# Samirez/Visual_odometry

Hardware: AMD Instinct MI355X
Metric: frame-pairs/sec (1280x720, 2000 ORB feats) (higher is better)
Workload: dtype u8+f32+f64; 1 GPU; seeded synthetic 1280x720 drone flight (256 distinct rendered views, closed loop), 2000 ORB features/frame, 8 levels = BASELINE config 2; chunk of 257 consecutive frames -> 256 pairs (k, k+1) per GPU per step, each frame detected once; detector=orb, distinct_rendered_frames=256, pair_stride=1, contexts_per_gpu=3, keypoint_order=cv2, poly_solver=fast, matcher=crosscheck, matcher_kernel=mfma_fp4, ransac=5-point, conf 0.99, 1 px, seed 2^64-1, <=1000 iters, parallelism=single GPU, pairs_ok_last_step=256

## Files before the change

### include/vo_hip.h

```cpp
#ifndef VO_HIP_H
#define VO_HIP_H
#include <stddef.h>
#include <stdint.h>

#ifdef __cplusplus
extern "C" {
#endif

#define VO_MAX_LEVELS 16

#define VO_OK                 0
#define VO_WARN_CAPACITY      1
#define VO_ERR_INVALID       -1
#define VO_ERR_HIP           -2
#define VO_ERR_TOO_FEW       -3
#define VO_ERR_NO_MODEL      -4
#define VO_ERR_NOT_CONFIGURED -5
#define VO_ERR_UNSUPPORTED    -7
#define VO_ERR_AMBIGUOUS      -6

typedef struct vo_ctx vo_ctx;

typedef struct {
    int32_t nfeatures;
// ... 71 lines not shown
typedef struct {
    int32_t match_mode;
    double  ratio;
    double  ransac_prob;
    double  ransac_thresh;
    int32_t ransac_max_iters;
    uint64_t ransac_seed;
    double  pose_dist_thresh;
    int32_t want_points;
} vo_pair_opts;

typedef struct {
    int32_t n_kp1, n_kp2, n_match, n_inl, n_good, status, ransac_iters, reserved;
    double  R[9], t[3], E[9];
} vo_pair_result;

int vo_batch_configure(vo_ctx* ctx, int h, int w, const vo_orb_params* params, int max_frames, int max_pairs);
int vo_frames_upload(vo_ctx* ctx, const uint8_t* frames, int F, int row_stride, int64_t frame_stride, int first_slot);
int vo_frames_upload_async(vo_ctx* ctx, const uint8_t* frames, int F, int row_stride, int64_t frame_stride, int first_slot);
int vo_frames_upload_color(vo_ctx* ctx, const uint8_t* frames, int F, int channels, int row_stride,
                           int64_t frame_stride, int first_slot);
int vo_frames_detect(vo_ctx* ctx, int first_slot, int F);
int vo_frames_detect_async(vo_ctx* ctx, int first_slot, int F);
int vo_batch_kp_capacity(vo_ctx* ctx);
int  vo_host_alloc(size_t bytes, void** out);
void vo_host_free(void* p);
int vo_frame_features(vo_ctx* ctx, int slot, float* kp_xy, float* kp_size, float* kp_angle, float* kp_response,
                      int32_t* kp_octave, uint8_t* desc, int cap, int32_t* n_out);
int vo_pairs_run(vo_ctx* ctx, const int32_t* pair_slots, int B, const double* K, const vo_pair_opts* opts,
                 vo_pair_result* results, double* X, int32_t x_cap);
int vo_pairs_run_async(vo_ctx* ctx, const int32_t* pair_slots, int B, const double* K, const vo_pair_opts* opts,
                       vo_pair_result* results, double* X, int32_t x_cap);
int vo_sync(vo_ctx* ctx);
int vo_detect_after(vo_ctx* ctx, vo_ctx* other);
int vo_pair_matches(vo_ctx* ctx, int pair, int32_t* qidx, int32_t* tidx, float* dist, uint8_t* inlier_mask,
                    int cap, int32_t* n_out);

#define VO_COMM_ID_BYTES 128
#define VO_RECORD_DOUBLES 16
int vo_comm_unique_id(uint8_t id[VO_COMM_ID_BYTES]);
int vo_comm_init(vo_ctx* ctx, const uint8_t id[VO_COMM_ID_BYTES], int rank, int world);
int vo_comm_destroy(vo_ctx* ctx);
int vo_comm_share(vo_ctx* ctx, vo_ctx* owner);
int vo_comm_info(vo_ctx* ctx, int32_t* n_ranks, int32_t* rank);
int vo_pairs_gather(vo_ctx* ctx, int B, double* gathered, int wait);
int vo_comm_allgather_f64(vo_ctx* ctx, const double* send, int n, double* recv);
// ... 223 lines not shown
```

### visual_odometry_amd/_lib.py

```python
from __future__ import annotations

import ctypes as C
import os

import numpy as np

_HERE = os.path.dirname(os.path.abspath(__file__))
LIB_PATH = os.environ.get("VO_HIP_LIBRARY") or os.path.join(_HERE, "libvo_hip.so")

VO_OK, VO_WARN_CAPACITY = 0, 1
VO_ERR_INVALID, VO_ERR_HIP, VO_ERR_TOO_FEW, VO_ERR_NO_MODEL, VO_ERR_NOT_CONFIGURED, VO_ERR_AMBIGUOUS = -1, -2, -3, -4, -5, -6
VO_ERR_UNSUPPORTED = -7
VO_STAGE_COUNT = 30
VO_COMM_ID_BYTES, VO_RECORD_DOUBLES = 128, 16
VO_BA_MAX_CAMERAS, VO_BA_MAX_FREE = 64, 16
VO_BA_LARGE_MAX_FREE = 512
VO_PGO_MAX_VERTICES, VO_PGO_MAX_LOOPS = 8192, 32
VO_STATS_HIST = 64


class OrbParams(C.Structure):
    _fields_ = [("nfeatures", C.c_int32), ("scale_factor", C.c_float), ("nlevels", C.c_int32),
                ("edge_threshold", C.c_int32), ("first_level", C.c_int32), ("wta_k", C.c_int32),
                ("score_type", C.c_int32), ("patch_size", C.c_int32), ("fast_threshold", C.c_int32)]
# ... 55 lines not shown
    "vo_orb_detect_and_compute": (C.c_int, [_P, _P, C.c_int, C.c_int, C.c_int, C.c_int, _P, _P, _P, _P, _P, _P, _P, C.c_int, _P]),
    "vo_match_hamming": (C.c_int, [_P, _P, C.c_int, _P, C.c_int, C.c_int, _P, _P, _P, _P]),
    "vo_match_l2": (C.c_int, [_P, _P, C.c_int, _P, C.c_int, C.c_int, C.c_int, _P, _P, _P, _P]),
    "vo_knn2_ratio_hamming": (C.c_int, [_P, _P, C.c_int, _P, C.c_int, C.c_double, _P, _P, _P, _P]),
    "vo_find_essential_ransac": (C.c_int, [_P, _P, _P, C.c_int, _P, C.c_double, C.c_double, C.c_int, C.c_uint64, _P, _P, _P, _P]),
    "vo_recover_pose": (C.c_int, [_P, _P, _P, _P, C.c_int, _P, C.c_double, _P, _P, _P, _P]),
    "vo_triangulate": (C.c_int, [_P, _P, _P, _P, _P, C.c_int, _P]),
    "vo_correspond_epilines": (C.c_int, [_P, _P, C.c_int, C.c_int, C.c_int, _P, _P]),
    "vo_pairs_epipolar": (C.c_int, [_P, C.c_int, _P, _P, _P, _P, _P, _P]),
    "vo_undistort_points": (C.c_int, [_P, _P, C.c_int, C.c_int, _P, _P, C.c_int, _P, _P, _P]),
    "vo_frames_undistort": (C.c_int, [_P, C.c_int, C.c_int, _P, _P, C.c_int]),
    "vo_packed_pyramid_bytes": (C.c_int64, [C.c_int, C.c_int, _P]),
    "vo_stage_pyramid": (C.c_int, [_P, _P, C.c_int, C.c_int, C.c_int, C.c_int, _P, _P]),
    "vo_stage_fast_scores": (C.c_int, [_P, _P, C.c_int, C.c_int, C.c_int, C.c_int, _P, _P]),
    "vo_stage_blur": (C.c_int, [_P, _P, C.c_int, C.c_int, C.c_int, C.c_int, _P, _P]),
    "vo_stage_five_point": (C.c_int, [_P, _P, _P, _P, _P]),
    "vo_batch_configure": (C.c_int, [_P, C.c_int, C.c_int, _P, C.c_int, C.c_int]),
    "vo_frames_upload": (C.c_int, [_P, _P, C.c_int, C.c_int, C.c_int64, C.c_int]),
    "vo_frames_upload_async": (C.c_int, [_P, _P, C.c_int, C.c_int, C.c_int64, C.c_int]),
    "vo_frames_upload_color": (C.c_int, [_P, _P, C.c_int, C.c_int, C.c_int, C.c_int64, C.c_int]),
    "vo_frames_detect": (C.c_int, [_P, C.c_int, C.c_int]),
    "vo_frames_detect_async": (C.c_int, [_P, C.c_int, C.c_int]),
    "vo_batch_kp_capacity": (C.c_int, [_P]),
    "vo_host_alloc": (C.c_int, [C.c_size_t, C.POINTER(_P)]),
    "vo_host_free": (None, [_P]),
    "vo_frame_features": (C.c_int, [_P, C.c_int, _P, _P, _P, _P, _P, _P, C.c_int, _P]),
    "vo_pairs_run": (C.c_int, [_P, _P, C.c_int, _P, _P, _P, _P, C.c_int32]),
    "vo_pairs_run_async": (C.c_int, [_P, _P, C.c_int, _P, _P, _P, _P, C.c_int32]),
    "vo_sync": (C.c_int, [_P]),
    "vo_set_matcher_kernel": (C.c_int, [_P, C.c_int]),
    "vo_set_poly_solver": (C.c_int, [_P, C.c_int]),
    "vo_set_pnp_refine": (C.c_int, [_P, C.c_int]),
    "vo_set_keypoint_order": (C.c_int, [_P, C.c_int]),
    "vo_stage_retain_best": (C.c_int, [_P, _P, C.c_int, C.c_int, _P, _P]),
    "vo_detect_after": (C.c_int, [_P, _P]),
    "vo_knn2_hamming": (C.c_int, [_P, _P, C.c_int, _P, C.c_int, _P, _P]),
    "vo_knn2_l2": (C.c_int, [_P, _P, C.c_int, _P, C.c_int, C.c_int, _P, _P]),
    "vo_knn2_ratio_l2": (C.c_int, [_P, _P, C.c_int, _P, C.c_int, C.c_int, C.c_double, _P, _P, _P, _P]),
    "vo_tracks_pnp_batch": (C.c_int, [_P, C.c_int, _P, C.c_int, C.c_double, C.c_double, C.c_uint64, C.c_double, _P, _P, _P, _P, _P]),
    "vo_slam_chain": (C.c_int, [_P, C.c_int, _P, _P, _P, _P, _P, _P, _P, _P, _P, _P, _P, _P, _P]),
    "vo_slam_map_size": (C.c_int, [_P, C.c_int, _P, _P, _P]),
    "vo_slam_map": (C.c_int, [_P, C.c_int, _P, _P, _P, _P, _P, _P, _P, _P]),
    "vo_slam_stream": (C.c_int, [_P, C.c_int, C.c_int, C.c_int, _P, _P, _P, _P, _P, _P, _P, _P, _P, _P, _P, _P, _P, _P, _P, _P]),
    "vo_slam_stream_restart": (C.c_int, [_P, C.c_int, C.c_int, C.c_int, _P, _P, _P, _P, _P, _P, _P, _P, _P, _P, _P, _P, _P, _P, _P, _P, _P, _P, _P, _P]),
    "vo_slam_chains": (C.c_int, [_P, C.c_int, _P, _P, _P, C.c_int, _P, _P, _P, _P, _P, _P, _P, _P, _P, _P, _P]),
    "vo_slam_chains_restart": (C.c_int, [_P, C.c_int, _P, _P, _P, C.c_int, _P, _P, _P, _P, _P, _P, _P, _P, _P, _P, _P, _P, _P, _P, _P]),
# ... 255 lines not shown
```

### visual_odometry_amd/csrc/orb_kernels.hip

```cpp
#include "vo_internal.h"
#include <type_traits>
#include <float.h>
#include <stdlib.h>

__constant__ __attribute__((aligned(16))) int8_t c_pattern[256 * 4] = {
#include "orb_pattern.inc"
};
__constant__ int c_umax[16] = {15, 15, 15, 15, 14, 14, 14, 13, 13, 12, 11, 10, 9, 8, 6, 3};
__constant__ int c_gauss7[7] = {18, 34, 49, 55, 49, 34, 18};


typedef short vo_s16x2 __attribute__((ext_vector_type(2)));
typedef unsigned short vo_u16x2 __attribute__((ext_vector_type(2)));
__device__ __forceinline__ uint32_t pk_sub16(uint32_t a, uint32_t b)
{
    return __builtin_bit_cast(uint32_t, __builtin_bit_cast(vo_s16x2, a) - __builtin_bit_cast(vo_s16x2, b));
}
__device__ __forceinline__ uint32_t pk_add16(uint32_t a, uint32_t b)
{
    return __builtin_bit_cast(uint32_t, __builtin_bit_cast(vo_s16x2, a) + __builtin_bit_cast(vo_s16x2, b));
}
__device__ __forceinline__ uint32_t pk_min16(uint32_t a, uint32_t b)
{
    return __builtin_bit_cast(uint32_t, __builtin_elementwise_min(__builtin_bit_cast(vo_s16x2, a), __builtin_bit_cast(vo_s16x2, b)));
// ... 79 lines not shown
        const int x = x4 + b;
        if (x < w) {
            const uint8_t* px = s + (size_t)x * channels;
            const int v = channels == 1 ? px[0] : (px[0] * 3735 + px[1] * 19235 + px[2] * 9798 + (1 << 14)) >> 15;
            out |= (uint32_t)v << (8 * b);
        }
    }
    if (x4 + 4 <= w && ((dstride | (int)(dframe & 3)) & 3) == 0) *(uint32_t*)d = out;
    else for (int b = 0; b < 4 && x4 + b < w; b++) d[b] = (uint8_t)(out >> (8 * b));
}

void launch_gray_plain(hipStream_t s, const uint8_t* src, int channels, int row_stride, int64_t frame_stride,
                       uint8_t* dst, int w, int h, int dstride, int64_t dframe, int F)
{
    dim3 grid(((w + 3) / 4 + 63) / 64, h, F);
    hipLaunchKernelGGL(k_gray_plain, grid, dim3(64), 0, s, src, channels, row_stride, frame_stride, dst, w, dstride, dframe);
}

__global__ void k_resize(uint8_t* pyr, int frame_bytes, LevelGeom src, LevelGeom dst, ResizeTab tab)
{
    const int f = blockIdx.z;
    const int dx0 = (blockIdx.x * blockDim.x + threadIdx.x) * 4;
    const int dy = blockIdx.y * blockDim.y + threadIdx.y;
    if (dx0 >= dst.stride || dy >= dst.h) return;
    const uint8_t* sp = pyr + (size_t)f * frame_bytes + src.off;
    uint8_t* dp = pyr + (size_t)f * frame_bytes + dst.off;
    int r0, r1; uint32_t w0 = 0, w1 = 0; bool edge;
    if (dy < tab.min_y)       { r0 = r1 = 0; edge = true; }
    else if (dy >= tab.max_y) { r0 = r1 = src.h - 1; edge = true; }
    else { r0 = tab.yofs[dy]; r1 = r0 + 1; edge = false; w1 = tab.yc1[dy]; w0 = 256 - w1; }
    const uint8_t* s0 = sp + (size_t)r0 * src.stride;
    const uint8_t* s1 = sp + (size_t)r1 * src.stride;
    uint32_t out = 0;
#pragma unroll
    for (int b = 0; b < 4; b++) {
        const int dx = dx0 + b;
        uint32_t v = 0;
        if (dx < dst.w) {
            uint32_t h0, h1;
            if (dx < tab.min_x)       { h0 = (uint32_t)s0[0] << 8; h1 = (uint32_t)s1[0] << 8; }
            else if (dx >= tab.max_x) { h0 = (uint32_t)s0[src.w - 1] << 8; h1 = (uint32_t)s1[src.w - 1] << 8; }
            else {
                const int xo = tab.xofs[dx];
                const uint32_t c1 = tab.xc1[dx], c0 = 256 - c1;
                h0 = c0 * s0[xo] + c1 * s0[xo + 1];
                h1 = c0 * s1[xo] + c1 * s1[xo + 1];
            }
            v = edge ? (h0 + 128u) >> 8 : (h0 * w0 + h1 * w1 + 32768u) >> 16;
            v = v > 255u ? 255u : v;
        }
        out |= v << (8 * b);
    }
    *(uint32_t*)(dp + (size_t)dy * dst.stride + dx0) = out;
}

template <int I, int N, typename F>
__device__ __forceinline__ void unroll_while(int n, F& f)
{
    if constexpr (I < N) {
        if (I < n) { f(std::integral_constant<int, I>{}); unroll_while<I + 1, N>(n, f); }
    }
}

#ifndef RS3_AHEAD
#define RS3_AHEAD 4
#endif
__global__ __launch_bounds__(RS2_THREADS) void k_resize_direct(uint8_t* pyr, int frame_bytes, LevelGeom src, LevelGeom dst, ResizeTab tab)
{
    const int f = blockIdx.z, tid = threadIdx.x, lane = tid & 63, wave = __builtin_amdgcn_readfirstlane(tid >> 6);
    const int tiles_x = (dst.w + RS2_WW - 1) / RS2_WW;
    const int bid = xcd_tile(blockIdx.x, gridDim.x);
    const int tx = bid % tiles_x, ty = bid / tiles_x;
    const int x0 = tx * RS2_WW, y0 = ty * RS2_TH;
    const int dy0 = y0 + wave * RS2_WH, dy1 = min(dy0 + RS2_WH, dst.h);
    if (dy0 >= dst.h) return;
    const uint8_t* sp = pyr + (size_t)f * frame_bytes + src.off;
    const int dx = x0 + 4 * lane;
    int o[4], c1[4];
#pragma unroll
    for (int i = 0; i < 4; i++) { const int xi = min(dx + i, dst.w - 1); o[i] = tab.xofs[xi]; c1[i] = tab.xc1[xi]; }
    static_assert(RS2_WH <= 64, "one lane per destination row of the strip");
    const int li = min(dy0 + lane, dst.h - 1);
    const int yo_l = tab.yofs[li];
    const uint32_t yw1 = tab.yc1[li];
    const int yc_l = (int)((256u - yw1) | (yw1 << 16));
    const int yo_first = __builtin_amdgcn_readlane(yo_l, 0), yo_last = __builtin_amdgcn_readlane(yo_l, dy1 - 1 - dy0);
    const int base = o[0] & ~3, sh = o[0] - base;
    const uint32_t q1 = (uint32_t)(o[1] - o[0]), q2 = (uint32_t)(o[2] - o[0]), q3 = (uint32_t)(o[3] - o[0]);
    const uint32_t sel_ae = 0x0c000c00u | (q2 << 16), sel_ao = 0x0c000c00u | q1 | (q3 << 16);
    const uint32_t sel_be = sel_ae + 0x00010001u, sel_bo = sel_ao + 0x00010001u;
    const uint32_t c1e = (uint32_t)c1[0] | ((uint32_t)c1[2] << 16), c1o = (uint32_t)c1[1] | ((uint32_t)c1[3] << 16);
    const int r_first = yo_first, r_end = yo_last + 2;
    static_assert((RS2_WH * 127 + 99) / 100 + 3 <= 32, "the emit mask of a strip fits 32 bits");
    uint32_t emask = dy0 + lane < dy1 ? 1u << (yo_l + 1 - r_first) : 0u;
#pragma unroll
    for (int d = 1; d < RS2_WH; d <<= 1) emask |= (uint32_t)__shfl_xor((int)emask, d, 64);
    emask = (uint32_t)__builtin_amdgcn_readfirstlane((int)emask);
    const __amdgpu_buffer_rsrc_t drs = __builtin_amdgcn_make_buffer_rsrc(pyr + (size_t)f * frame_bytes + dst.off, 0, dst.stride * dst.h, 0x00020000);
    uint32_t out = (uint32_t)(dy0 * dst.stride + dx);
    const bool col_ok = dx < dst.stride;
    const int hmax = src.h - 1;
    uint32_t w[RS3_AHEAD][3];
#pragma unroll
    for (int u = 0; u < RS3_AHEAD; u++) {
        const uint32_t* q = (const uint32_t*)(sp + ((uint32_t)(min(r_first + u, hmax) * src.stride) + (uint32_t)base));
        w[u][0] = q[0]; w[u][1] = q[1]; w[u][2] = q[2];
    }
    int dyi = 0;
    uint32_t pe = 0, po = 0;
    const int nrows = r_end - r_first;
    constexpr int RS3_MAXR = (RS2_WH * 127 + 99) / 100 + 3;
    auto row = [&](auto ic) {
        constexpr int i = decltype(ic)::value, u = i % RS3_AHEAD;
        const uint32_t w0 = w[u][0], w1 = w[u][1], w2 = w[u][2];
        {
            const uint32_t* q = (const uint32_t*)(sp + ((uint32_t)(min(r_first + i + RS3_AHEAD, hmax) * src.stride) + (uint32_t)base));
            w[u][0] = q[0]; w[u][1] = q[1]; w[u][2] = q[2];
        }
        const uint32_t x0w = __builtin_amdgcn_alignbyte(w1, w0, (uint32_t)sh), x1w = __builtin_amdgcn_alignbyte(w2, w1, (uint32_t)sh);
        const uint32_t a_e = __builtin_amdgcn_perm(x1w, x0w, sel_ae), a_o = __builtin_amdgcn_perm(x1w, x0w, sel_ao);
        const uint32_t b_e = __builtin_amdgcn_perm(x1w, x0w, sel_be), b_o = __builtin_amdgcn_perm(x1w, x0w, sel_bo);
        const vo_u16x2 h_e = __builtin_bit_cast(vo_u16x2, c1e) * __builtin_bit_cast(vo_u16x2, pk_sub16(b_e, a_e)) + __builtin_bit_cast(vo_u16x2, a_e << 8);
        const vo_u16x2 h_o = __builtin_bit_cast(vo_u16x2, c1o) * __builtin_bit_cast(vo_u16x2, pk_sub16(b_o, a_o)) + __builtin_bit_cast(vo_u16x2, a_o << 8);
// ... 6 lines not shown
            const uint32_t d2 = __builtin_amdgcn_udot2(__builtin_bit_cast(vo_u16x2, __builtin_amdgcn_perm(ce, pe, 0x07060302u)), wv, 32768u, false);
            const uint32_t d1 = __builtin_amdgcn_udot2(__builtin_bit_cast(vo_u16x2, __builtin_amdgcn_perm(co, po, 0x05040100u)), wv, 32768u, false);
            const uint32_t d3 = __builtin_amdgcn_udot2(__builtin_bit_cast(vo_u16x2, __builtin_amdgcn_perm(co, po, 0x07060302u)), wv, 32768u, false);
            const uint32_t t01 = __builtin_amdgcn_perm(d1, d0, 0x0c0c0602u), t23 = __builtin_amdgcn_perm(d3, d2, 0x0c0c0602u);
            __builtin_amdgcn_raw_buffer_store_b32(__builtin_amdgcn_perm(t23, t01, 0x05040100u), drs, col_ok && emit ? out : 0xfffffff0u, 0, 0);
            out += emit ? (uint32_t)dst.stride : 0u;
            dyi += emit ? 1 : 0;
        }
        pe = ce; po = co;
    };
    unroll_while<0, RS3_MAXR>(nrows, row);
}

void launch_resize(hipStream_t s, uint8_t* pyr, const PyrGeom& g, int level, const ResizeTab& tab, int F)
{
    const LevelGeom& d = g.lv[level];
    if (tab.direct) {
        dim3 grid(((d.w + RS2_WW - 1) / RS2_WW) * ((d.h + RS2_TH - 1) / RS2_TH), 1, F);
        hipLaunchKernelGGL(k_resize_direct, grid, dim3(RS2_THREADS), 0, s, pyr, g.frame_bytes, g.lv[level - 1], d, tab);
        return;
    }
    dim3 block(64, 4), grid((d.stride / 4 + 63) / 64, (d.h + 3) / 4, F);
    hipLaunchKernelGGL(k_resize, grid, block, 0, s, pyr, g.frame_bytes, g.lv[level - 1], d, tab);
}

__global__ __launch_bounds__(256) void k_resize_linear(const uint8_t* src, int sw, int sh, int cn, int sstride, int64_t sframe,
                                                       uint8_t* dst, int dw, int dh, int dstride, int64_t dframe,
                                                       const int* xofs, const short2* xa, const int* yofs, const short2* yb, int area2)
{
    const int i = blockIdx.x * 256 + threadIdx.x, dy = blockIdx.y;
    if (i >= dw * cn) return;
    const int dx = i / cn, k = i - dx * cn;
    const uint8_t* s = src + (size_t)blockIdx.z * sframe;
    uint8_t* d = dst + (size_t)blockIdx.z * dframe + (size_t)dy * dstride + i;
    if (area2) {
        const uint8_t* q = s + (size_t)(2 * dy) * sstride + (size_t)(2 * dx) * cn + k;
        *d = (uint8_t)((q[0] + q[cn] + q[sstride] + q[sstride + cn] + 2) >> 2);
        return;
    }
    const int sy0 = min(max(yofs[dy], 0), sh - 1), sy1 = min(max(yofs[dy] + 1, 0), sh - 1);
    const int sx = xofs[dx], sx1 = min(sx + 1, sw - 1);
    const short2 a = xa[dx], b = yb[dy];
    const uint8_t* p0 = s + (size_t)sy0 * sstride; const uint8_t* p1 = s + (size_t)sy1 * sstride;
    const int r0 = p0[sx * cn + k] * a.x + p0[sx1 * cn + k] * a.y;
    const int r1 = p1[sx * cn + k] * a.x + p1[sx1 * cn + k] * a.y;
    const int v = (((b.x * (r0 >> 4)) >> 16) + ((b.y * (r1 >> 4)) >> 16) + 2) >> 2;
// ... 1350 lines not shown
```

### visual_odometry_amd/csrc/vo_api.hip

```cpp
#include "vo_host.h"

static const char* k_stage_names[VO_STAGE_COUNT] = {
    "gray", "pyramid_resize", "fast_score_nms", "select_fast", "harris", "select_harris", "ic_angle",
    "gaussian_blur", "rbrief", "match_nn", "match_select", "essential_ransac", "recover_pose",
    "triangulate", "misc", "reserved", "sift_scale_space", "sift_extrema", "sift_refine_orient", "sift_sort_unique",
    "sift_descriptor", "cv2_keypoint_order", "trajectory_gather", "reserved2", "slam_ba_prepare", "slam_bundle_adjust", "slam_filter",
    "slam_camera_limit", "slam_map_statistics", "undistort_points"};

static void clear_last_run(vo_ctx* ctx) { ctx->last = LastRun(); }

static void slam_stream_slots_written(vo_ctx* ctx, int first, int n)
{
    for (int k = first < 0 ? 0 : first; k < first + n && k < (int)ctx->undistorted.size(); k++) ctx->undistorted[(size_t)k] = 0;
    SlamStream& st = ctx->stream_map;
    if (st.live && st.anchor >= first && st.anchor < first + n) st.touched = true;
    for (SlamStream::Seq& q : st.seq)
        if (st.live && q.anchor >= first && q.anchor < first + n) q.touched = true;
}

void prof_collect(vo_ctx* c)
{
    for (int i = 0; i < c->n_ev; i++) {
        float ms = 0;
        if (hipEventElapsedTime(&ms, c->ev[i][0], c->ev[i][1]) == hipSuccess) {
// ... 74 lines not shown
    const double scale = 1.0 / inv_scale;
    int minofst = 0, maxofst = dsize;
    for (int val = 0; val < dsize; val++) {
        volatile double fval = scale * ((double)val + 0.5);
        fval = fval - 0.5;
        const double fv = fval;
        const int ival = cv_floor_d(fv);
        ofs[val] = 0; c1[val] = 0;
        if (ival >= 0 && ssize > 1) {
            if (ival < ssize - 1) {
                ofs[val] = ival;
                volatile double fr = fv - (double)ival;
                fr = fr * 256.0;
                c1[val] = (uint16_t)lrint((double)fr);
            } else {
                ofs[val] = ssize - 1;
                if (val < maxofst) maxofst = val;
            }
        } else if (val + 1 > minofst) minofst = val + 1;
    }
    *pmin = minofst; *pmax = maxofst;
}

static hipError_t alloc_pairbuf(DevList& mem, PairBuf& pb, int P, int cap, bool with_pose_mask)
{
    hipError_t e;
    const size_t pc = (size_t)P * cap;
    pb = PairBuf{};
#define A_(field, n) if ((e = mem.alloc(&pb.field, (n))) != hipSuccess) return e
    A_(slots, (size_t)P * 2); A_(nn_idx, pc * 2); A_(nn_dist, pc * 2); A_(nn_idx2, pc); A_(nn_dist2, pc);
    A_(m_q, pc); A_(m_t, pc); A_(m_d, pc); A_(m_count, (size_t)P);
    A_(px1, pc * 2); A_(px2, pc * 2); A_(xn1, pc * 2); A_(xn2, pc * 2);
    A_(mask, pc); A_(models, (size_t)P * 64 * 90); A_(pose_state, (size_t)P);
    A_(in1, pc * 2); A_(in2, pc * 2); A_(ipx1, pc * 2); A_(ipx2, pc * 2);
    A_(res, (size_t)P); A_(X, pc * 4);
    if (with_pose_mask) { A_(pose_mask, pc); }
    if (const size_t n = nn_colkey_ints(P, cap)) { A_(nn_colkey, n); }
#undef A_
    return hipSuccess;
}

static int alloc_cv2(vo_ctx* ctx)
{
    if (ctx->cv2_ready) return VO_OK;
    const PyrGeom& g = ctx->g;
    Cv2Buf& cb = ctx->cv2;
// ... 173 lines not shown
        drop_map(ctx);
    drop_places(ctx);
        ctx->undistorted.clear();
        return VO_OK;
    }
    HIPCHK(hipStreamSynchronize(ctx->stream));
    free_config(ctx);
    PyrGeom g;
    rc = make_geometry(ctx, h, w, params, &g);
    if (rc) return rc;
    ctx->g = g; ctx->h = h; ctx->w = w; ctx->params = *params;
    ctx->max_frames = max_frames; ctx->max_pairs = max_pairs;

    size_t tab_ints = 0, tab_u16 = 0;
    for (int l = 1; l < g.nlevels; l++) { tab_ints += g.lv[l].w + g.lv[l].h; tab_u16 += g.lv[l].w + g.lv[l].h; }
    std::vector<int> hofs(tab_ints + 1);
    std::vector<uint16_t> hc(tab_u16 + 1);
    const size_t int_bytes = (tab_ints + 1) * sizeof(int);
    DevList& m = ctx->orb_mem;
    uint8_t* tab_mem = nullptr;
    HIPCHK(m.alloc(&tab_mem, int_bytes + (tab_u16 + 1) * sizeof(uint16_t) + 64));
    int* d_ofs = (int*)tab_mem;
    uint16_t* d_c = (uint16_t*)(tab_mem + int_bytes);
    size_t oi = 0;
    for (int l = 1; l < g.nlevels; l++) {
        ResizeTab& t = ctx->tabs[l];
        const LevelGeom &s = g.lv[l - 1], &d = g.lv[l];
        build_lin_tab(s.w, d.w, &hofs[oi], &hc[oi], &t.min_x, &t.max_x);
        t.xofs = d_ofs + oi; t.xc1 = d_c + oi; oi += d.w;
        build_lin_tab(s.h, d.h, &hofs[oi], &hc[oi], &t.min_y, &t.max_y);
        t.yofs = d_ofs + oi; t.yc1 = d_c + oi; oi += d.h;
        {
            const int* xo = &hofs[oi - d.h - d.w]; const int* yo = &hofs[oi - d.h];
            bool ok = true;
            for (int x = 0; x + 3 < d.w && ok; x++) ok = xo[x + 3] - xo[x] <= 4;
            for (int y = 0; y + 1 < d.h && ok; y++) ok = yo[y + 1] > yo[y];
            for (int y0 = 0; y0 < d.h && ok; y0 += RS2_WH) { const int yl = (y0 + RS2_WH < d.h ? y0 + RS2_WH : d.h) - 1; ok = yo[yl] + 2 - yo[y0] <= (RS2_WH * 127 + 99) / 100 + 3; }
            t.direct = ok ? 1 : 0;
        }
    }
    HIPCHK(hipMemcpy(d_ofs, hofs.data(), int_bytes, hipMemcpyHostToDevice));
    HIPCHK(hipMemcpy(d_c, hc.data(), (tab_u16 + 1) * sizeof(uint16_t), hipMemcpyHostToDevice));

    const size_t F = (size_t)max_frames, fb = (size_t)g.frame_bytes;
    HIPCHK(m.alloc(&ctx->pyr, F * fb + 256));
    HIPCHK(m.alloc(&ctx->blur, F * fb));
    HIPCHK(m.alloc(&ctx->score, F * fb));
    HIPCHK(hipMemset(ctx->pyr, 0, F * fb));
    FrameFeat& ff = ctx->ff;
    HIPCHK(m.alloc(&ff.cand_pos, F * g.cand_total)); HIPCHK(m.alloc(&ff.cand_resp, F * g.cand_total));
    HIPCHK(m.alloc(&ff.cand_count, F * VO_MAX_LEVELS));
    HIPCHK(m.alloc(&ff.kp_pos, F * g.kp_cap)); HIPCHK(m.alloc(&ff.kp_level, F * g.kp_cap));
    HIPCHK(m.alloc(&ff.kp_resp, F * g.kp_cap)); HIPCHK(m.alloc(&ff.kp_angle, F * g.kp_cap));
    HIPCHK(m.alloc(&ff.kp_xy, F * g.kp_cap * 2)); HIPCHK(m.alloc(&ff.kp_size, F * g.kp_cap));
    HIPCHK(m.alloc(&ff.desc, F * g.kp_cap * 32));
    HIPCHK(m.alloc(&ctx->desc_x, F * (size_t)desc_x_rows(g.kp_cap) * 256));
    HIPCHK(hipMemset(ctx->desc_x, 0xFF, F * (size_t)desc_x_rows(g.kp_cap) * 256));
    HIPCHK(m.alloc(&ff.kp_count, F)); HIPCHK(m.alloc(&ff.flags, F));
    HIPCHK(m.alloc(&ff.hist, F * VO_MAX_LEVELS * 256));
    HIPCHK(m.alloc(&ff.tile_list, F * (size_t)g.ftiles_total * FAST_LISTCAP));
    HIPCHK(m.alloc(&ff.tile_count, F * (size_t)g.ftiles_total));
    HIPCHK(m.alloc(&ctx->sel_thr, F * VO_MAX_LEVELS));
    HIPCHK(m.alloc(&ctx->har_kept, F * VO_MAX_LEVELS));
// ... 108 lines not shown
    if (ctx->prof) prof_collect(ctx);
    return VO_OK;
}

static int run_detect(vo_ctx* ctx, int first_slot, int F, int upto)
{
    const PyrGeom& g = ctx->g;
    hipStream_t s = ctx->stream;
    uint8_t* pyr = ctx->pyr + (size_t)first_slot * g.frame_bytes;
    uint8_t* blur = ctx->blur + (size_t)first_slot * g.frame_bytes;
    uint8_t* score = ctx->score + (size_t)first_slot * g.frame_bytes;
    FrameFeat ff = ctx->ff;
    ff.cand_pos += (size_t)first_slot * g.cand_total; ff.cand_resp += (size_t)first_slot * g.cand_total;
    ff.cand_count += (size_t)first_slot * VO_MAX_LEVELS;
    ff.kp_pos += (size_t)first_slot * g.kp_cap; ff.kp_level += (size_t)first_slot * g.kp_cap;
    ff.kp_resp += (size_t)first_slot * g.kp_cap; ff.kp_angle += (size_t)first_slot * g.kp_cap;
    ff.kp_xy += (size_t)first_slot * g.kp_cap * 2; ff.kp_size += (size_t)first_slot * g.kp_cap;
    ff.desc += (size_t)first_slot * g.kp_cap * 32;
    ff.kp_count += first_slot; ff.flags += first_slot;
    ff.hist += (size_t)first_slot * VO_MAX_LEVELS * 256;
    ff.tile_list += (size_t)first_slot * g.ftiles_total * FAST_LISTCAP; ff.tile_count += (size_t)first_slot * g.ftiles_total;
    {
        StageTimer t(ctx, ST_RESIZE);
        for (int l = 1; l < g.nlevels; l++) launch_resize(s, pyr, g, l, ctx->tabs[l], F);
    }
    if (upto < 1) return VO_OK;
    const bool cv2 = ctx->kp_order == 1 && ctx->cv2_ready;
    Cv2Buf cb = ctx->cv2;
    if (cv2) {
        const size_t fo = (size_t)first_slot;
        cb.all_pos += fo * cb.all_total; cb.all_resp += fo * cb.all_total; cb.work += fo * cb.all_total;
        cb.all_cand += fo * cb.all_total; cb.lpos += fo * cb.all_total; cb.rpos += fo * cb.all_total;
        cb.all_count += fo * VO_MAX_LEVELS; cb.chunk_count += fo * g.sel_chunks_total;
    }
    {
        StageTimer t(ctx, ST_MISC);
        HIPCHK(hipMemsetAsync(ff.hist, 0, (size_t)F * VO_MAX_LEVELS * 256 * sizeof(uint32_t), s));
        if (upto < 2) {
            HIPCHK(hipMemsetAsync(ff.flags, 0, (size_t)F * sizeof(int), s));
            HIPCHK(hipMemsetAsync(ff.cand_count, 0, (size_t)F * VO_MAX_LEVELS * sizeof(int), s));
            if (cv2) HIPCHK(hipMemsetAsync(cb.all_count, 0, (size_t)F * VO_MAX_LEVELS * sizeof(int), s));
        }
    }
    { StageTimer t(ctx, ST_FAST); launch_fast(s, pyr, score, ff.hist, g, F, upto < 2 ? nullptr : ff.tile_list, ff.tile_count); }
    if (upto < 2) return VO_OK;
    { StageTimer t(ctx, ST_SELECT_FAST); launch_select_fast(s, g, ff, F, ctx->sel_thr + (size_t)first_slot * VO_MAX_LEVELS, ctx->sel_chunk_count + (size_t)first_slot * g.sel_chunks_total, ff.tile_list, ff.tile_count, cv2 ? &cb : nullptr); }
    if (g.score_type == 0) { StageTimer t(ctx, ST_HARRIS); launch_harris(s, pyr, g, ff, F); }
    { StageTimer t(ctx, ST_SELECT_HARRIS); launch_select_harris(s, g, ff, F, ctx->har_thr + (size_t)first_slot * VO_MAX_LEVELS, ctx->har_kept + (size_t)first_slot * VO_MAX_LEVELS); }
    if (cv2) {
        StageTimer t(ctx, ST_CV2_ORDER);
        launch_cv2_order(s, g, ff, cb, F, ctx->har_kept + (size_t)first_slot * VO_MAX_LEVELS);
    }
    { StageTimer t(ctx, ST_BLUR); launch_blur(s, pyr, blur, g, F); }
    {
        StageTimer t(ctx, ST_BRIEF);
        const int cx = desc_x_rows(g.kp_cap);
        const int fp4 = descx_begin_write(ctx, first_slot, F);
        launch_brief(s, pyr, blur, g, ff, F, ctx->desc_x + (size_t)first_slot * cx * 256, cx, fp4);
    }
    return VO_OK;
}

extern "C" int vo_batch_kp_capacity(vo_ctx* ctx)
{
    if (!ctx) return 0;
    const Batch b = batch(ctx);
    return b.ready ? b.kp_cap : 0;
}

extern "C" int vo_host_alloc(size_t bytes, void** out)
{
    if (!out) return VO_ERR_INVALID;
    *out = nullptr;
    return hipHostMalloc(out, bytes ? bytes : 1, hipHostMallocDefault) == hipSuccess ? VO_OK : VO_ERR_HIP;
}

extern "C" void vo_host_free(void* p)
{
    if (p) (void)hipHostFree(p);
}

static int detect_enqueue(vo_ctx* ctx, int first_slot, int F)
// ... 2114 lines not shown
```

### visual_odometry_amd/csrc/vo_internal.h

```cpp
#pragma once
#include <hip/hip_runtime.h>
#include <stdint.h>
#include "../../include/vo_hip.h"

enum {
    ST_GRAY = 0, ST_RESIZE, ST_FAST, ST_SELECT_FAST, ST_HARRIS, ST_SELECT_HARRIS, ST_ANGLE,
    ST_BLUR, ST_BRIEF, ST_MATCH_NN, ST_MATCH_SELECT, ST_RANSAC, ST_POSE, ST_TRIANGULATE,
    ST_MISC, ST_RESERVED, ST_SIFT_SCALE, ST_SIFT_EXTREMA, ST_SIFT_ORIENT, ST_SIFT_SORT, ST_SIFT_DESC, ST_CV2_ORDER, ST_GATHER, ST_RESERVED2,
    ST_SLAM_PREPARE, ST_SLAM_BA, ST_SLAM_FILTER, ST_SLAM_LIMIT, ST_SLAM_STATS, ST_UNDISTORT
};

struct LevelGeom {
    int w, h, stride, off;
    int quota;
    float scale;
    int ftile_base, ftiles_x;
    int fox, foy;
    int dtile_base, dtiles_x;
    int btile_base, btiles_x;
    int cand_off, cand_cap;
    int sel_chunk_base;
};

struct PyrGeom {
    int nlevels, frame_bytes;
    int edge, fast_thr, score_type, nfeatures;
    int ftiles_total, btiles_total, dtiles_total;
    int cand_total, kp_cap;
    int sel_chunks_total;
    LevelGeom lv[VO_MAX_LEVELS];
};

#define RS2_WW 256
#define RS2_WH 16
#ifndef RS2_WAVES
#define RS2_WAVES 4
#endif
#define RS2_THREADS (64 * RS2_WAVES)
#define RS2_TH (RS2_WAVES * RS2_WH)

struct ResizeTab {
    const int* xofs; const uint16_t* xc1;
    const int* yofs; const uint16_t* yc1;
    int min_x, max_x, min_y, max_y;
    int direct;
};

#ifndef FAST_TW
#define FAST_TW 112
#endif
#ifndef FAST_TH
#define FAST_TH 20
#endif
#define BLUR_TW 128
#ifndef BLUR_TH
#define BLUR_TH 48
#endif
#define FAST_LISTCAP ((FAST_TW / 2) * (FAST_TH / 2))

struct FrameFeat {
    uint32_t* cand_pos;
    float*    cand_resp;
    int*      cand_count;
    uint32_t* kp_pos;
    int*      kp_level;
    float*    kp_resp;
    float*    kp_angle;
    float*    kp_xy;
    float*    kp_size;
// ... 53 lines not shown

struct RansacParams {
    double prob, thresh_px;
    int max_iters;
    uint64_t seed;
    double K[9];
    double dist_thresh;
    int dk_early;
};

const char* rccl_load(void);
const char* rccl_unique_id(uint8_t* id128);
const char* rccl_comm_init(void** comm, const uint8_t* id128, int rank, int world);
void rccl_comm_destroy(void* comm);
const char* rccl_comm_count(void* comm, int* n);
const char* rccl_all_gather_f64(void* comm, const double* send, double* recv, size_t count, hipStream_t s);
void launch_pack_records(hipStream_t s, const vo_pair_result* res, int B, int valid, double* rec);

void launch_gray(hipStream_t s, const uint8_t* src, int channels, int row_stride, int64_t frame_stride,
                 uint8_t* pyr, const PyrGeom& g, int F);
void launch_gray_plain(hipStream_t s, const uint8_t* src, int channels, int row_stride, int64_t frame_stride,
                       uint8_t* dst, int w, int h, int dstride, int64_t dframe, int F);
void launch_resize(hipStream_t s, uint8_t* pyr, const PyrGeom& g, int level, const ResizeTab& tab, int F);
void launch_fast(hipStream_t s, const uint8_t* pyr, uint8_t* score, uint32_t* hist, const PyrGeom& g, int F,
                 uint32_t* tile_list, int* tile_count);
void launch_select_fast(hipStream_t s, const PyrGeom& g, FrameFeat ff, int F, int* thr, int* chunk_count,
                        const uint32_t* tile_list, const int* tile_count, const Cv2Buf* cb);
void launch_harris(hipStream_t s, const uint8_t* pyr, const PyrGeom& g, FrameFeat ff, int F);
void launch_cv2_order(hipStream_t s, const PyrGeom& g, FrameFeat ff, Cv2Buf cb, int F, const int* kept);
void launch_retain_raw(hipStream_t s, const float* resp, int n, int n_points, uint2* a, uint32_t* lpos, uint32_t* rpos,
                       int* order, int* n_out);
void launch_select_harris(hipStream_t s, const PyrGeom& g, FrameFeat ff, int F, float* thr, int* kept);
void launch_resize_linear(hipStream_t st, const uint8_t* src, int sw, int sh, int cn, int sstride, int64_t sframe,
                          uint8_t* dst, int dw, int dh, int dstride, int64_t dframe,
                          const int* xofs, const void* xa, const int* yofs, const void* yb, int area2, int F);
void launch_resize_area(hipStream_t st, const uint8_t* src, int cn, int sstride, uint8_t* dst, int dw, int dh, int dstride,
                        int isx, int isy, const int* xsi, const float* xal, const int* xst, const int* ysi, const float* yal, const int* yst);
#define SIFT_IMG_BORDER 5
#define SIFT_MAX_INTERP_STEPS 5
#define SIFT_MAX_OCT 16
#define SIFT_MAX_TAPS 64
struct SiftGeom {
    int nOct, nLayers;
    int w[SIFT_MAX_OCT], h[SIFT_MAX_OCT], stride[SIFT_MAX_OCT];
    size_t plane[SIFT_MAX_OCT];
    size_t goff[SIFT_MAX_OCT];
// ... 359 lines not shown
```

Before: 109,000 frame-pairs/s.

## Fuse two consecutive pyramid resize levels into one kernel via LDS staging

```diff
diff --git a/include/vo_hip.h b/include/vo_hip.h
--- a/include/vo_hip.h
+++ b/include/vo_hip.h
@@ -117,6 +117,9 @@
                            int64_t frame_stride, int first_slot);
 int vo_frames_detect(vo_ctx* ctx, int first_slot, int F);
 int vo_frames_detect_async(vo_ctx* ctx, int first_slot, int F);
+int64_t vo_pyramid_layout(vo_ctx* ctx, int32_t* layout);
+int vo_frames_pyramid_raw(vo_ctx* ctx, int slot, uint8_t* out);
+int vo_pyramid_fill(vo_ctx* ctx, int value);
 int vo_batch_kp_capacity(vo_ctx* ctx);
 int  vo_host_alloc(size_t bytes, void** out);
 void vo_host_free(void* p);
diff --git a/visual_odometry_amd/_lib.py b/visual_odometry_amd/_lib.py
--- a/visual_odometry_amd/_lib.py
+++ b/visual_odometry_amd/_lib.py
@@ -101,6 +101,9 @@
     "vo_frames_detect": (C.c_int, [_P, C.c_int, C.c_int]),
     "vo_frames_detect_async": (C.c_int, [_P, C.c_int, C.c_int]),
     "vo_batch_kp_capacity": (C.c_int, [_P]),
+    "vo_pyramid_layout": (C.c_int64, [_P, _P]),
+    "vo_frames_pyramid_raw": (C.c_int, [_P, C.c_int, _P]),
+    "vo_pyramid_fill": (C.c_int, [_P, C.c_int]),
     "vo_host_alloc": (C.c_int, [C.c_size_t, C.POINTER(_P)]),
     "vo_host_free": (None, [_P]),
     "vo_frame_features": (C.c_int, [_P, C.c_int, _P, _P, _P, _P, _P, _P, C.c_int, _P]),
diff --git a/visual_odometry_amd/csrc/orb_kernels.hip b/visual_odometry_amd/csrc/orb_kernels.hip
--- a/visual_odometry_amd/csrc/orb_kernels.hip
+++ b/visual_odometry_amd/csrc/orb_kernels.hip
@@ -125,7 +125,7 @@
     const int f = blockIdx.z;
     const int dx0 = (blockIdx.x * blockDim.x + threadIdx.x) * 4;
     const int dy = blockIdx.y * blockDim.y + threadIdx.y;
-    if (dx0 >= dst.stride || dy >= dst.h) return;
+    if (dx0 >= dst.w || dy >= dst.h) return;
     const uint8_t* sp = pyr + (size_t)f * frame_bytes + src.off;
     uint8_t* dp = pyr + (size_t)f * frame_bytes + dst.off;
     int r0, r1; uint32_t w0 = 0, w1 = 0; bool edge;
@@ -154,7 +154,9 @@
         }
         out |= v << (8 * b);
     }
-    *(uint32_t*)(dp + (size_t)dy * dst.stride + dx0) = out;
+    uint8_t* d = dp + (size_t)dy * dst.stride + dx0;
+    if (dx0 + 4 <= dst.w) *(uint32_t*)d = out;
+    else for (int b = 0; dx0 + b < dst.w; b++) d[b] = (uint8_t)(out >> (8 * b));
 }
 
 template <int I, int N, typename F>
@@ -178,10 +180,10 @@
     const int dy0 = y0 + wave * RS2_WH, dy1 = min(dy0 + RS2_WH, dst.h);
     if (dy0 >= dst.h) return;
     const uint8_t* sp = pyr + (size_t)f * frame_bytes + src.off;
-    const int dx = x0 + 4 * lane;
+    const int dx = x0 + 4 * lane, dxs = dx < dst.w && dx + 4 > dst.w ? dst.w - 4 : dx;
     int o[4], c1[4];
 #pragma unroll
-    for (int i = 0; i < 4; i++) { const int xi = min(dx + i, dst.w - 1); o[i] = tab.xofs[xi]; c1[i] = tab.xc1[xi]; }
+    for (int i = 0; i < 4; i++) { const int xi = min(dxs + i, dst.w - 1); o[i] = tab.xofs[xi]; c1[i] = tab.xc1[xi]; }
     static_assert(RS2_WH <= 64, "one lane per destination row of the strip");
     const int li = min(dy0 + lane, dst.h - 1);
     const int yo_l = tab.yofs[li];
@@ -200,8 +202,8 @@
     for (int d = 1; d < RS2_WH; d <<= 1) emask |= (uint32_t)__shfl_xor((int)emask, d, 64);
     emask = (uint32_t)__builtin_amdgcn_readfirstlane((int)emask);
     const __amdgpu_buffer_rsrc_t drs = __builtin_amdgcn_make_buffer_rsrc(pyr + (size_t)f * frame_bytes + dst.off, 0, dst.stride * dst.h, 0x00020000);
-    uint32_t out = (uint32_t)(dy0 * dst.stride + dx);
-    const bool col_ok = dx < dst.stride;
+    uint32_t out = (uint32_t)(dy0 * dst.stride + dxs);
+    const bool col_ok = dx < dst.w;
     const int hmax = src.h - 1;
     uint32_t w[RS3_AHEAD][3];
 #pragma unroll
@@ -254,6 +256,162 @@
     }
     dim3 block(64, 4), grid((d.stride / 4 + 63) / 64, (d.h + 3) / 4, F);
     hipLaunchKernelGGL(k_resize, grid, block, 0, s, pyr, g.frame_bytes, g.lv[level - 1], d, tab);
+}
+
+struct RsCols { uint32_t base, sh, sel_ae, sel_ao, sel_be, sel_bo, c1e, c1o; };
+
+__device__ __forceinline__ RsCols rs_cols(const int (&o)[4], const int (&c1)[4])
+{
+    RsCols k;
+    k.base = (uint32_t)(o[0] & ~3); k.sh = (uint32_t)o[0] - k.base;
+    const uint32_t q1 = (uint32_t)(o[1] - o[0]), q2 = (uint32_t)(o[2] - o[0]), q3 = (uint32_t)(o[3] - o[0]);
+    k.sel_ae = 0x0c000c00u | (q2 << 16); k.sel_ao = 0x0c000c00u | q1 | (q3 << 16);
+    k.sel_be = k.sel_ae + 0x00010001u; k.sel_bo = k.sel_ao + 0x00010001u;
+    k.c1e = (uint32_t)c1[0] | ((uint32_t)c1[2] << 16); k.c1o = (uint32_t)c1[1] | ((uint32_t)c1[3] << 16);
+    return k;
+}
+
+__device__ __forceinline__ void rs_hblend(uint32_t w0, uint32_t w1, uint32_t w2, const RsCols& k, uint32_t& ce, uint32_t& co)
+{
+    const uint32_t x0w = __builtin_amdgcn_alignbyte(w1, w0, k.sh), x1w = __builtin_amdgcn_alignbyte(w2, w1, k.sh);
+    const uint32_t a_e = __builtin_amdgcn_perm(x1w, x0w, k.sel_ae), a_o = __builtin_amdgcn_perm(x1w, x0w, k.sel_ao);
+    const uint32_t b_e = __builtin_amdgcn_perm(x1w, x0w, k.sel_be), b_o = __builtin_amdgcn_perm(x1w, x0w, k.sel_bo);
+    const vo_u16x2 h_e = __builtin_bit_cast(vo_u16x2, k.c1e) * __builtin_bit_cast(vo_u16x2, pk_sub16(b_e, a_e)) + __builtin_bit_cast(vo_u16x2, a_e << 8);
+    const vo_u16x2 h_o = __builtin_bit_cast(vo_u16x2, k.c1o) * __builtin_bit_cast(vo_u16x2, pk_sub16(b_o, a_o)) + __builtin_bit_cast(vo_u16x2, a_o << 8);
+    ce = __builtin_bit_cast(uint32_t, h_e); co = __builtin_bit_cast(uint32_t, h_o);
+}
+
+__device__ __forceinline__ uint32_t rs_vblend(uint32_t ce, uint32_t pe, uint32_t co, uint32_t po, vo_u16x2 wv)
+{
+    const uint32_t d0 = __builtin_amdgcn_udot2(__builtin_bit_cast(vo_u16x2, __builtin_amdgcn_perm(ce, pe, 0x05040100u)), wv, 32768u, false);
+    const uint32_t d2 = __builtin_amdgcn_udot2(__builtin_bit_cast(vo_u16x2, __builtin_amdgcn_perm(ce, pe, 0x07060302u)), wv, 32768u, false);
+    const uint32_t d1 = __builtin_amdgcn_udot2(__builtin_bit_cast(vo_u16x2, __builtin_amdgcn_perm(co, po, 0x05040100u)), wv, 32768u, false);
+    const uint32_t d3 = __builtin_amdgcn_udot2(__builtin_bit_cast(vo_u16x2, __builtin_amdgcn_perm(co, po, 0x07060302u)), wv, 32768u, false);
+    const uint32_t t01 = __builtin_amdgcn_perm(d1, d0, 0x0c0c0602u), t23 = __builtin_amdgcn_perm(d3, d2, 0x0c0c0602u);
+    return __builtin_amdgcn_perm(t23, t01, 0x05040100u);
+}
+
+__device__ __forceinline__ int rs_edge_col(int x, int w) { return x < w && x + 4 > w ? w - 4 : x; }
+
+__device__ __forceinline__ uint32_t rs_or32(uint32_t m)
+{
+#pragma unroll
+    for (int d = 1; d < 32; d <<= 1) m |= (uint32_t)__shfl_xor((int)m, d, 64);
+    return (uint32_t)__builtin_amdgcn_readfirstlane((int)m);
+}
+__device__ __forceinline__ uint64_t rs_or64(uint64_t m) { return rs_or32((uint32_t)m) | ((uint64_t)rs_or32((uint32_t)(m >> 32)) << 32); }
+
+#define RP_LROW 512
+__global__ __launch_bounds__(RP_THREADS) void k_resize_pair(uint8_t* pyr, int frame_bytes, LevelGeom l0, LevelGeom l1, LevelGeom l2, ResizeTab t1, ResizeTab t2)
+{
+    __shared__ __attribute__((aligned(16))) uint8_t s_rows[RP_WAVES][2][RP_LROW];
+    const int f = blockIdx.z, tid = threadIdx.x, lane = tid & 63, wave = __builtin_amdgcn_readfirstlane(tid >> 6);
+    const int tiles_x = RP_TILES_X(l2.w);
+    const int bid = xcd_tile(blockIdx.x, gridDim.x);
+    const int tx = bid % tiles_x, ty = bid / tiles_x;
+    const int x2_0 = tx * RP_WW, y2_0 = ty * RP_TH + wave * RP_WH;
+    if (y2_0 >= l2.h) return;
+    const int y2_1 = min(y2_0 + RP_WH, l2.h);
+    const bool last_x = tx == tiles_x - 1, last_y = y2_1 == l2.h;
+    const int x1_0 = t2.xofs[x2_0] & ~3;
+    const int x1_own = last_x ? l1.w : min(t2.xofs[last_x ? 0 : x2_0 + RP_WW] & ~3, l1.w);
+    const int r1_first = t2.yofs[y2_0], r1_need = t2.yofs[y2_1 - 1] + 2;
+    const int n1 = min(r1_need, l1.h) - r1_first;
+    const int own_n = (last_y ? l1.h : t2.yofs[last_y ? 0 : y2_1]) - r1_first;
+    const uint8_t* sp = pyr + (size_t)f * frame_bytes + l0.off;
+    const int x1 = x1_0 + 4 * lane, x2 = x2_0 + 4 * lane, x1s = rs_edge_col(x1, l1.w), x2s = rs_edge_col(x2, l2.w);
+    const int x2_lim = last_x ? l2.w - 1 : x2_0 + RP_WW - 1;
+    const uint32_t lsh = 8u * (uint32_t)(x1 - x1s);
+    int o[4], c1[4];
+#pragma unroll
+    for (int i = 0; i < 4; i++) { const int xi = min(x1s + i, l1.w - 1); o[i] = t1.xofs[xi]; c1[i] = t1.xc1[xi]; }
+    const RsCols ka = rs_cols(o, c1);
+#pragma unroll
+    for (int i = 0; i < 4; i++) { const int xi = min(x2s + i, x2_lim); o[i] = t2.xofs[xi] - x1_0; c1[i] = t2.xc1[xi]; }
+    const RsCols kb = rs_cols(o, c1);
+    static_assert(RP_N1MAX < 32 && RP_N0MAX <= 64 && RP_WH <= 32, "the emit masks of a strip fit 64 / 32 bits, its rows lanes 0 .. 31");
+    const int li1 = min(r1_first + lane, l1.h - 1), li2 = min(y2_0 + lane, l2.h - 1);
+    const int yo1_l = t1.yofs[li1], yo2_l = t2.yofs[li2];
+    const uint32_t yw1 = t1.yc1[li1], yw2 = t2.yc1[li2];
+    const int yc1_l = (int)((256u - yw1) | (yw1 << 16)), yc2_l = (int)((256u - yw2) | (yw2 << 16));
+    const int r0_first = __builtin_amdgcn_readlane(yo1_l, 0), r0_end = __builtin_amdgcn_readlane(yo1_l, n1 - 1) + 2;
+    uint64_t emask1 = rs_or64(lane < n1 ? 1ull << (yo1_l + 1 - r0_first) : 0ull);
+    uint32_t emask2 = rs_or32(lane < y2_1 - y2_0 ? 1u << (yo2_l + 1 - r1_first) : 0u);
+    const __amdgpu_buffer_rsrc_t drs1 = __builtin_amdgcn_make_buffer_rsrc(pyr + (size_t)f * frame_bytes + l1.off, 0, l1.stride * l1.h, 0x00020000);
+    const __amdgpu_buffer_rsrc_t drs2 = __builtin_amdgcn_make_buffer_rsrc(pyr + (size_t)f * frame_bytes + l2.off, 0, l2.stride * l2.h, 0x00020000);
+    uint32_t out1 = (uint32_t)(r1_first * l1.stride + x1s), out2 = (uint32_t)(y2_0 * l2.stride + x2s);
+    const bool col1_ok = x1 < x1_own;
+    const bool col2_ok = x2 < l2.w && (last_x || lane < RP_WW / 4);
+    uint8_t* const lrow = &s_rows[wave][0][0];
+    const int hmax = l0.h - 1;
+    uint32_t w[RS3_AHEAD][3];
+#pragma unroll
+    for (int u = 0; u < RS3_AHEAD; u++) {
+        const uint32_t* q = (const uint32_t*)(sp + ((uint32_t)(min(r0_first + u, hmax) * l0.stride) + ka.base));
+        w[u][0] = q[0]; w[u][1] = q[1]; w[u][2] = q[2];
+    }
+    int j1 = 0, j2 = 0;
+    uint32_t pe = 0, po = 0, pe2 = 0, po2 = 0;
+    uint32_t vb[3] = {0, 0, 0};
+    auto stage_b_read = [&](int j) {
+        const uint32_t* q = (const uint32_t*)(lrow + (j & 1) * RP_LROW + kb.base);
+        vb[0] = q[0]; vb[1] = q[1]; vb[2] = q[2];
+    };
+    auto stage_b = [&]() {
+        const uint32_t v0 = vb[0], v1 = vb[1], v2 = vb[2];
+        uint32_t ce, co;
+        rs_hblend(v0, v1, v2, kb, ce, co);
+        const bool emit = emask2 & 1u;
+        emask2 >>= 1;
+        const vo_u16x2 wv = __builtin_bit_cast(vo_u16x2, __builtin_amdgcn_readlane(yc2_l, j2));
+        __builtin_amdgcn_raw_buffer_store_b32(rs_vblend(ce, pe2, co, po2, wv), drs2, col2_ok && emit ? out2 : 0xfffffff0u, 0, 0);
+        out2 += emit ? (uint32_t)l2.stride : 0u;
+        j2 += emit ? 1 : 0;
+        pe2 = ce; po2 = co;
+    };
+    const int nrows = r0_end - r0_first;
+    auto row = [&](auto ic) {
+        constexpr int i = decltype(ic)::value, u = i % RS3_AHEAD;
+        const uint32_t w0 = w[u][0], w1 = w[u][1], w2 = w[u][2];
+        {
+            const uint32_t* q = (const uint32_t*)(sp + ((uint32_t)(min(r0_first + i + RS3_AHEAD, hmax) * l0.stride) + ka.base));
+            w[u][0] = q[0]; w[u][1] = q[1]; w[u][2] = q[2];
+        }
+        uint32_t ce, co;
+        rs_hblend(w0, w1, w2, ka, ce, co);
+        const bool emit = emask1 & 1u;
+        emask1 >>= 1;
+        const vo_u16x2 wv = __builtin_bit_cast(vo_u16x2, __builtin_amdgcn_readlane(yc1_l, j1));
+        const uint32_t px = rs_vblend(ce, pe, co, po, wv);
+        __builtin_amdgcn_raw_buffer_store_b32(px, drs1, col1_ok && emit && j1 < own_n ? out1 : 0xfffffff0u, 0, 0);
+        if (emit) {
+            *(uint32_t*)(lrow + (j1 & 1) * RP_LROW + 4 * lane) = px >> lsh;
+            __builtin_amdgcn_wave_barrier();
+            stage_b_read(j1);
+            stage_b();
+            __builtin_amdgcn_wave_barrier();
+        }
+        out1 += emit ? (uint32_t)l1.stride : 0u;
+        j1 += emit ? 1 : 0;
+        pe = ce; po = co;
+    };
+    unroll_while<0, RP_N0MAX>(nrows, row);
+    if (r1_need > l1.h) stage_b();
+}
+
+void launch_resize_pairs(hipStream_t s, uint8_t* pyr, const PyrGeom& g, const ResizeTab* tabs, int F)
+{
+    for (int l = 1; l < g.nlevels; ) {
+        if (l + 1 < g.nlevels && tabs[l + 1].pair) {
+            const LevelGeom& d = g.lv[l + 1];
+            dim3 grid(RP_TILES_X(d.w) * ((d.h + RP_TH - 1) / RP_TH), 1, F);
+            hipLaunchKernelGGL(k_resize_pair, grid, dim3(RP_THREADS), 0, s, pyr, g.frame_bytes, g.lv[l - 1], g.lv[l], d, tabs[l], tabs[l + 1]);
+            l += 2;
+        } else {
+            launch_resize(s, pyr, g, l, tabs[l], F);
+            l += 1;
+        }
+    }
 }
 
 __global__ __launch_bounds__(256) void k_resize_linear(const uint8_t* src, int sw, int sh, int cn, int sstride, int64_t sframe,
diff --git a/visual_odometry_amd/csrc/vo_api.hip b/visual_odometry_amd/csrc/vo_api.hip
--- a/visual_odometry_amd/csrc/vo_api.hip
+++ b/visual_odometry_amd/csrc/vo_api.hip
@@ -120,6 +120,27 @@
     *pmin = minofst; *pmax = maxofst;
 }
 
+static bool resize_pair_fits(const LevelGeom& l1, const LevelGeom& l2, const int* yo1, const int* xo2, const int* yo2)
+{
+    if (xo2[0] != 0 || yo2[0] != 0) return false;
+    for (int x = 0; x + 1 < l2.w; x++) if (xo2[x + 1] < xo2[x] || xo2[x + 1] > xo2[x] + 2) return false;
+    for (int y = 0; y + 1 < l2.h; y++) if (yo2[y + 1] <= yo2[y] || yo2[y + 1] > yo2[y] + 2) return false;
+    for (int tx = 0; tx < RP_TILES_X(l2.w); tx++) {
+        const bool last = tx == RP_TILES_X(l2.w) - 1;
+        const int x0 = tx * RP_WW, xl = last ? l2.w - 1 : x0 + RP_WW - 1, x1_0 = xo2[x0] & ~3;
+        if (xo2[xl] + 1 - x1_0 > 255) return false;
+        if (last && x1_0 + 256 < l1.w) return false;
+    }
+    for (int y0 = 0; y0 < l2.h; y0 += RP_WH) {
+        const bool last = y0 + RP_WH >= l2.h;
+        const int yl = last ? l2.h - 1 : y0 + RP_WH - 1, r1_first = yo2[y0];
+        const int r1_end = yo2[yl] + 2 < l1.h ? yo2[yl] + 2 : l1.h;
+        if (r1_end - r1_first > RP_N1MAX || yo1[r1_end - 1] + 2 - yo1[r1_first] > RP_N0MAX) return false;
+        if (last ? r1_end != l1.h : yo2[y0 + RP_WH] > r1_end) return false;
+    }
+    return true;
+}
+
 static hipError_t alloc_pairbuf(DevList& mem, PairBuf& pb, int P, int cap, bool with_pose_mask)
 {
     hipError_t e;
@@ -339,9 +360,10 @@
     HIPCHK(m.alloc(&tab_mem, int_bytes + (tab_u16 + 1) * sizeof(uint16_t) + 64));
     int* d_ofs = (int*)tab_mem;
     uint16_t* d_c = (uint16_t*)(tab_mem + int_bytes);
-    size_t oi = 0;
+    size_t oi = 0, xpos[VO_MAX_LEVELS] = {}, ypos[VO_MAX_LEVELS] = {};
     for (int l = 1; l < g.nlevels; l++) {
         ResizeTab& t = ctx->tabs[l];
+        t.pair = 0;
         const LevelGeom &s = g.lv[l - 1], &d = g.lv[l];
         build_lin_tab(s.w, d.w, &hofs[oi], &hc[oi], &t.min_x, &t.max_x);
         t.xofs = d_ofs + oi; t.xc1 = d_c + oi; oi += d.w;
@@ -349,13 +371,17 @@
         t.yofs = d_ofs + oi; t.yc1 = d_c + oi; oi += d.h;
         {
             const int* xo = &hofs[oi - d.h - d.w]; const int* yo = &hofs[oi - d.h];
-            bool ok = true;
+            bool ok = d.w >= 4;
             for (int x = 0; x + 3 < d.w && ok; x++) ok = xo[x + 3] - xo[x] <= 4;
             for (int y = 0; y + 1 < d.h && ok; y++) ok = yo[y + 1] > yo[y];
             for (int y0 = 0; y0 < d.h && ok; y0 += RS2_WH) { const int yl = (y0 + RS2_WH < d.h ? y0 + RS2_WH : d.h) - 1; ok = yo[yl] + 2 - yo[y0] <= (RS2_WH * 127 + 99) / 100 + 3; }
             t.direct = ok ? 1 : 0;
         }
-    }
+        xpos[l] = oi - d.h - d.w; ypos[l] = oi - d.h;
+    }
+    for (int l = 2; l < g.nlevels; l++)
+        ctx->tabs[l].pair = ctx->tabs[l - 1].direct && ctx->tabs[l].direct &&
+                            resize_pair_fits(g.lv[l - 1], g.lv[l], &hofs[ypos[l - 1]], &hofs[xpos[l]], &hofs[ypos[l]]) ? 1 : 0;
     HIPCHK(hipMemcpy(d_ofs, hofs.data(), int_bytes, hipMemcpyHostToDevice));
     HIPCHK(hipMemcpy(d_c, hc.data(), (tab_u16 + 1) * sizeof(uint16_t), hipMemcpyHostToDevice));
 
@@ -510,7 +536,7 @@
     ff.tile_list += (size_t)first_slot * g.ftiles_total * FAST_LISTCAP; ff.tile_count += (size_t)first_slot * g.ftiles_total;
     {
         StageTimer t(ctx, ST_RESIZE);
-        for (int l = 1; l < g.nlevels; l++) launch_resize(s, pyr, g, l, ctx->tabs[l], F);
+        launch_resize_pairs(s, pyr, g, ctx->tabs, F);
     }
     if (upto < 1) return VO_OK;
     const bool cv2 = ctx->kp_order == 1 && ctx->cv2_ready;
@@ -546,6 +572,42 @@
         const int fp4 = descx_begin_write(ctx, first_slot, F);
         launch_brief(s, pyr, blur, g, ff, F, ctx->desc_x + (size_t)first_slot * cx * 256, cx, fp4);
     }
+    return VO_OK;
+}
+
+extern "C" int64_t vo_pyramid_layout(vo_ctx* ctx, int32_t* layout)
+{
+    if (!ctx) return VO_ERR_INVALID;
+    const Batch b = batch(ctx);
+    if (!b.ready || b.sift) FAIL(VO_ERR_NOT_CONFIGURED, "vo_pyramid_layout needs an ORB batch configuration");
+    if (!layout) FAIL(VO_ERR_INVALID, "layout is NULL");
+    for (int l = 0; l < ctx->g.nlevels; l++) {
+        const LevelGeom& lv = ctx->g.lv[l];
+        layout[4 * l] = lv.w; layout[4 * l + 1] = lv.h; layout[4 * l + 2] = lv.stride; layout[4 * l + 3] = lv.off;
+    }
+    return ctx->g.frame_bytes;
+}
+
+extern "C" int vo_frames_pyramid_raw(vo_ctx* ctx, int slot, uint8_t* out)
+{
+    if (!ctx) return VO_ERR_INVALID;
+    const Batch b = batch(ctx);
+    if (!b.ready || b.sift) FAIL(VO_ERR_NOT_CONFIGURED, "vo_frames_pyramid_raw needs an ORB batch configuration");
+    if (!out || slot < 0 || slot >= b.max_frames) FAIL(VO_ERR_INVALID, "slot out of range");
+    HIPCHK(hipSetDevice(ctx->device));
+    HIPCHK(hipStreamSynchronize(ctx->stream));
+    HIPCHK(hipMemcpy(out, ctx->pyr + (size_t)slot * ctx->g.frame_bytes, (size_t)ctx->g.frame_bytes, hipMemcpyDeviceToHost));
+    return VO_OK;
+}
+
+extern "C" int vo_pyramid_fill(vo_ctx* ctx, int value)
+{
+    if (!ctx) return VO_ERR_INVALID;
+    const Batch b = batch(ctx);
+    if (!b.ready || b.sift) FAIL(VO_ERR_NOT_CONFIGURED, "vo_pyramid_fill needs an ORB batch configuration");
+    HIPCHK(hipSetDevice(ctx->device));
+    HIPCHK(hipMemsetAsync(ctx->pyr, value, (size_t)b.max_frames * ctx->g.frame_bytes, ctx->stream));
+    HIPCHK(hipStreamSynchronize(ctx->stream));
     return VO_OK;
 }
 
diff --git a/visual_odometry_amd/csrc/vo_internal.h b/visual_odometry_amd/csrc/vo_internal.h
--- a/visual_odometry_amd/csrc/vo_internal.h
+++ b/visual_odometry_amd/csrc/vo_internal.h
@@ -44,7 +44,19 @@
     const int* yofs; const uint16_t* yc1;
     int min_x, max_x, min_y, max_y;
     int direct;
-};
+    int pair;
+};
+
+#define RP_WW 192
+#ifndef RP_WH
+#define RP_WH 14
+#endif
+#define RP_WAVES 4
+#define RP_THREADS (64 * RP_WAVES)
+#define RP_TH (RP_WAVES * RP_WH)
+#define RP_TILES_X(w) ((w) > RP_WW + 3 ? ((w) - 3 + RP_WW - 1) / RP_WW : 1)
+#define RP_N1MAX ((RP_WH * 127 + 99) / 100 + 3)
+#define RP_N0MAX ((RP_N1MAX * 127 + 99) / 100 + 3)
 
 #ifndef FAST_TW
 #define FAST_TW 112
@@ -144,6 +156,7 @@
 void launch_gray_plain(hipStream_t s, const uint8_t* src, int channels, int row_stride, int64_t frame_stride,
                        uint8_t* dst, int w, int h, int dstride, int64_t dframe, int F);
 void launch_resize(hipStream_t s, uint8_t* pyr, const PyrGeom& g, int level, const ResizeTab& tab, int F);
+void launch_resize_pairs(hipStream_t s, uint8_t* pyr, const PyrGeom& g, const ResizeTab* tabs, int F);
 void launch_fast(hipStream_t s, const uint8_t* pyr, uint8_t* score, uint32_t* hist, const PyrGeom& g, int F,
                  uint32_t* tile_list, int* tile_count);
 void launch_select_fast(hipStream_t s, const PyrGeom& g, FrameFeat ff, int F, int* thr, int* chunk_count,
```

After: 108,800 frame-pairs/s. About the same (-0.1%).
